# ctu-mrs/mrs_optic_flow

Measured on AMD Instinct MI355X. Metric: frame_pairs_per_s_fft_phase_corr, higher is better.
Workload: dtype f32

## Files before the change

### __graft_entry__.py

```python
from __future__ import annotations

import os
import subprocess
import sys

ROOT = os.path.dirname(os.path.abspath(__file__))


def build() -> None:
    jobs = f"-j{max(1, min(8, os.cpu_count() or 1))}"
    subprocess.check_call(["make", "-C", os.path.join(ROOT, "mrs_optic_flow_amd", "csrc"), "-s", jobs])
    subprocess.check_call(["make", "-C", os.path.join(ROOT, "oracle"), "-s", "all"])
    subprocess.check_call(["make", "-C", os.path.join(ROOT, "tests", "cpp"), "-s"])
    subprocess.check_call(["make", "-C", os.path.join(ROOT, "tests", "cpp_quality"), "-s"])
    subprocess.check_call(["make", "-C", os.path.join(ROOT, "tests", "cpp_gate"), "-s"])
    subprocess.check_call(["make", "-C", os.path.join(ROOT, "tests", "cpp_bm_quality"), "-s"])
    if ROOT not in sys.path:
        sys.path.insert(0, ROOT)
    import mrs_optic_flow_amd

    assert mrs_optic_flow_amd.FftMethod is not None
    subprocess.check_call([sys.executable, "-c", "from mrs_optic_flow_amd import _capi; _capi.load()"], cwd=ROOT,
                          env=dict(os.environ, MOF_NO_TORCH_PRELOAD="1"))


def smoke() -> None:
    if ROOT not in sys.path:
        sys.path.insert(0, ROOT)
    sys.path.insert(0, os.path.join(ROOT, "tests"))
    import torch
    import numpy as np

    import oracle_lib
    from mrs_optic_flow_amd import FastSpacedBMMethod, FftMethod, synth

    assert torch.cuda.is_available(), "smoke() needs a GPU"
    h, w = 160, 224
    cur, prev, shifts, _ = synth.batch_np(2, h, w, s=5, classes=False, k0=1)
    fm = FftMethod(sample_point_size=64, frame_shape=(h, w), grid=(3, 2), origin=(1, 1), stride=(79, 47))
    got = fm.process_batch_device(torch.from_numpy(cur).cuda(), torch.from_numpy(prev).cuda()).cpu().numpy()
    lay = oracle_lib.fft_layout(w, h, 64, 3, 2, (1, 1), (79, 47))
    for k in range(2):
        want, _ = oracle_lib.fft_process(cur[k], prev[k], lay, 64)
        assert np.allclose(got[k], want, rtol=0, atol=1e-4, equal_nan=True), (got[k], want)
        assert np.allclose(np.nanmedian(got[k], axis=0), shifts[k], rtol=0, atol=0.5)
    for n, gx, gy, stride in ((60, 3, 2, (70, 50)), (37, 4, 3, (40, 39))):
# ... 64 lines not shown
```

### mrs_optic_flow_amd/csrc/mof_capi.hip

```cpp

#include "mof.h"

#include <hip/hip_runtime.h>

#include <atomic>
#include <cmath>
#include <cstdarg>
#include <cstdio>
#include <cstdlib>
#include <cstring>
#include <memory>
#include <mutex>
#include <new>
#include <vector>

#include "capi_graph.hpp"
#include "host_pipe.hpp"
#include "mof_kernels.h"
#include "pc_launch.hpp"

#include "pc_gate_kernel.hip"

namespace {
thread_local char g_err[512] = "";
// ... 421 lines not shown
  if (c->peak_model == MOF_PEAK_OCL && c->search_radius < 0) return fail(MOF_ERR_BAD_ARG, "search_radius must be >= 0");
  return MOF_OK;
}

static void fft_destroy_now(void* p) {
  mof_fft_engine* e = static_cast<mof_fft_engine*>(p);
  mof::RelaxedCapture relaxed;
  (void)hipSetDevice(e->cfg.device);
  if (e->stream) (void)hipStreamSynchronize(e->stream);
  e->fence.wait_idle();
  e->gate_fence.wait_idle();
  delete e;
}
struct FftDestroyNow {
  void operator()(mof_fft_engine* e) const { fft_destroy_now(e); }
};

int mof_fft_create(const mof_fft_config* cfg, mof_fft_engine** out) try {
  if (!out) return fail(MOF_ERR_BAD_ARG, "null out");
  *out = nullptr;
  int rc = validate_fft(cfg);
  if (rc) return rc;
  rc = mof::select_device(cfg->device);
  if (rc) return rc;
  mof::RelaxedCapture relaxed;
  const size_t res = (size_t)cfg->grid_x * cfg->grid_y * 2;
  std::unique_ptr<mof_fft_engine, FftDestroyNow> e(new (std::nothrow) mof_fft_engine());
  if (!e) return fail(MOF_ERR_NO_MEMORY, "out of host memory");
  e->cfg = *cfg;
  e->frame_bytes = (size_t)cfg->frame_width * cfg->frame_height;
  if (!fft_route(*cfg, &e->plan, &e->route))
    return fail(MOF_ERR_UNSUPPORTED, "no plan for patch_size %d", cfg->patch_size);
  const FftRoute& r = e->route;
  const std::vector<float> tw = mof::twiddle_table(r.m);
  HIP_TRY(e->stream.create());
  HIP_TRY(mof::upload(e->d_twiddles, tw, e->stream));
  for (auto& frame : e->d_frames) {
    HIP_TRY(frame.alloc(e->frame_bytes));
    HIP_TRY(mof::fill_on(e->stream, frame, 0, e->frame_bytes));
  }
  HIP_TRY(mof::alloc_all(e->d_out, res, e->h_out, res, e->d_quality, res, e->h_quality, res, e->h_stage, e->frame_bytes));
  if (r.half_m > 0 || r.video == FftRoute::HALF_SEQ) HIP_TRY(mof::pc_configure_half(r.half_m > 0 ? r.half_m : r.video_m));
  if (r.family == FftRoute::LARGE) {
    HIP_TRY(e->fence.create());
    HIP_TRY(large_alloc(e.get(), cfg->grid_x * cfg->grid_y));
  } else if (r.family == FftRoute::PLANNED) {
    HIP_TRY(mof::pc_configure_generic());
  } else {
    HIP_TRY(mof::pc_configure(r.m));
  }
  if (r.video == FftRoute::SEQ) HIP_TRY(mof::pc_configure_sequence());
  if (r.video == FftRoute::SEQ_HALF) HIP_TRY(mof::pc_configure_sequence_half(r.m));
  *out = e.release();
  return MOF_OK;
} catch (const std::bad_alloc&) {
  return fail(MOF_ERR_NO_MEMORY, "mof_fft_create: out of host memory");
}

const char* mof_fft_kernel_variant(const mof_fft_engine* e) {
  if (!e) return "";
  const FftRoute& r = e->route;
  return r.half_m > 0 ? "planned-half"
                      : (r.family == FftRoute::LARGE ? "planned-large"
                                                     : (r.family == FftRoute::PLANNED ? "planned" : "stockham"));
}

void mof_fft_destroy(mof_fft_engine* e) {
// ... 650 lines not shown
```

### mrs_optic_flow_amd/csrc/mof_kernels.h

```cpp
#pragma once

#include <hip/hip_runtime.h>
#include <stdint.h>

#include <vector>

namespace mof {

struct PcArgs {
  const uint8_t* cur;
  const uint8_t* prev;
  size_t cur_stride;
  size_t prev_stride;
  size_t pitch;
  int grid_x, grid_y;
  int origin_x, origin_y;
  int stride_x, stride_y;
  int total;
  int stagger_div, stagger_units;
  int channels;
  int downscale;
  int peak_model;
  int search_radius;
  double max_px_speed_sq;
// ... 36 lines not shown
  int n_cand;
  const float* twiddles;
  int m, n;
  int mode;
  double M_log;
  double max_px_speed_sq;
  double* out;
  const int* flags;
  const float* cdc;
  int peak_model;
  int search_radius;
  double* quality;
  double min_response;
};
size_t pcl_zh_floats(const PcPlan& pl);
int pcl_candidates(const PcPlan& pl);
hipError_t launch_pcl_rows(const PclSrc& src, const PcPlan& pl, const float* twiddles, float* zh, size_t zh_stride, int* flags,
                           int n_images, int channels, int downscale, hipStream_t stream);
hipError_t launch_pcl_cols(const float* zh_prev, const float* zh_cur, size_t zh_stride, const PcPlan& pl, const float* twiddles,
                           float* Dt, float* cdc, const int* flags, int n_pairs, hipStream_t stream, int peak_model = 0);
hipError_t launch_pcl_peak(const PclFinal& a, const PcPlan& pl, int n_pairs, hipStream_t stream, bool candidates_done = false);
hipError_t launch_pcl_cdc(const float* zh_prev, const float* zh_cur, size_t zh_stride, int m, float* cdc, int n_pairs, hipStream_t stream);

bool pc_half_supported(int m);
int pc_half_workgroups_per_cu(int m);
hipError_t pc_configure_half(int m);
hipError_t launch_pc_half(const PcArgs& a, int m, int n, int n_pairs, hipStream_t stream);
bool pc_half_sequence_supported(int m);
hipError_t launch_pc_half_sequence(const PcArgs& a, int m, int n, int n_pairs, int run, hipStream_t stream);

bool pc_patch_size_supported(int n);
hipError_t pc_configure(int patch_size);
hipError_t launch_pc_field(const PcArgs& a, int patch_size, int n_pairs, hipStream_t stream);
bool pc_sequence_supported(int patch_size);
hipError_t pc_configure_sequence();
hipError_t launch_pc_sequence(const PcArgs& a, int n_pairs, int run, hipStream_t stream);
bool pc_sequence_half_supported(int patch_size);
hipError_t pc_configure_sequence_half(int patch_size);
hipError_t launch_pc_sequence_half(const PcArgs& a, int patch_size, int n_pairs, int run, hipStream_t stream);
hipError_t pc_configure_120();
hipError_t launch_pc_field_120(const PcArgs& a, int n_pairs, hipStream_t stream);
hipError_t launch_pc_response_gate(double* out, const double* quality, size_t n_patches, double min_response, hipStream_t stream);

struct BmArgs {
  const uint8_t* cur;
  const uint8_t* prev;
  size_t cur_stride, prev_stride, pitch;
  int grid_x, grid_y;
  int block, step, radius;
  int low_contrast_rule;
  int channels;
  int8_t* dx;
  int8_t* dy;
  int8_t* mode;
};

struct BmQArgs {
  uint32_t* quality = nullptr;
  uint32_t max_min_sad = 0xffffffffu, min_sad_range = 0u;
};
constexpr int BM_INVALID = -128;
inline bool bm_gate_armed(const BmQArgs& q) { return q.max_min_sad != 0xffffffffu || q.min_sad_range != 0u; }

bool bm_config_supported(int block, int radius);
bool bm_scan_plan(int block, int step, int radius, int grid_x, bool quality, int out[4]);
hipError_t launch_bm_scan(const BmArgs& a, const BmQArgs& q, int n_pairs, hipStream_t stream);
// ... 124 lines not shown
```

### mrs_optic_flow_amd/csrc/pc_common.hpp

```cpp
#pragma once

#include <hip/hip_runtime.h>
#include <stdint.h>

#include "mof_kernels.h"

namespace mof {
namespace {

struct cf {
  float x, y;
};

__device__ __forceinline__ cf cmul(cf a, cf b) { return {a.x * b.x - a.y * b.y, a.x * b.y + a.y * b.x}; }
__device__ __forceinline__ cf cadd(cf a, cf b) { return {a.x + b.x, a.y + b.y}; }
__device__ __forceinline__ cf csub(cf a, cf b) { return {a.x - b.x, a.y - b.y}; }
__device__ __forceinline__ cf mul_mi(cf a) { return {a.y, -a.x}; }

template <int R>
__device__ __forceinline__ void butterfly(cf* v);

template <>
__device__ __forceinline__ void butterfly<2>(cf* v) {
  cf a = v[0], b = v[1];
  v[0] = cadd(a, b);
  v[1] = csub(a, b);
}

template <>
__device__ __forceinline__ void butterfly<4>(cf* v) {
  cf a = cadd(v[0], v[2]), b = csub(v[0], v[2]);
  cf c = cadd(v[1], v[3]), d = mul_mi(csub(v[1], v[3]));
  v[0] = cadd(a, c);
  v[1] = cadd(b, d);
  v[2] = csub(a, c);
  v[3] = csub(b, d);
}

// ... 130 lines not shown
  const cf w[22] = {{1.f, 0.f}, {c1, -s1}, {c2, -s2}, {c3, -s3}, {h, -h}, {s3, -c3}, {s2, -c2}, {s1, -c1}, {0.f, -1.f},
                    {-s1, -c1}, {-s2, -c2}, {-s3, -c3}, {-h, -h}, {-c3, -s3}, {-c2, -s2}, {-c1, -s1}, {-1.f, 0.f},
                    {-c1, s1}, {-c2, s2}, {-c3, s3}, {-h, h}, {-s3, c3}};
  cf t[8][4];
#pragma unroll
  for (int n2 = 0; n2 < 8; ++n2) {
    cf a[4] = {v[n2], v[8 + n2], v[16 + n2], v[24 + n2]};
    butterfly<4>(a);
#pragma unroll
    for (int k1 = 0; k1 < 4; ++k1) t[n2][k1] = (n2 * k1 == 0) ? a[k1] : cmul(a[k1], w[n2 * k1]);
  }
#pragma unroll
  for (int k1 = 0; k1 < 4; ++k1) {
    cf b[8] = {t[0][k1], t[1][k1], t[2][k1], t[3][k1], t[4][k1], t[5][k1], t[6][k1], t[7][k1]};
    butterfly<8>(b);
#pragma unroll
    for (int k2 = 0; k2 < 8; ++k2) v[k1 + 4 * k2] = b[k2];
  }
}

__device__ __forceinline__ void wave_sync() {
  __builtin_amdgcn_fence(__ATOMIC_RELEASE, "wavefront");
  __builtin_amdgcn_wave_barrier();
  __builtin_amdgcn_fence(__ATOMIC_ACQUIRE, "wavefront");
}

__device__ __forceinline__ cf lds_read(const cf* p) {
  typedef float f2 __attribute__((ext_vector_type(2)));
  typedef const volatile f2 __attribute__((address_space(3))) * lds_f2_ptr;
  const f2 t = *(lds_f2_ptr)(p);
  return {t.x, t.y};
}

struct Best {
  float v;
  int idx;
};
__device__ __forceinline__ Best better(Best a, Best b) {
  return (b.v > a.v || (b.v == a.v && b.idx < a.idx)) ? b : a;
}

__device__ __forceinline__ int wave_lane() { return (int)__builtin_amdgcn_mbcnt_hi(~0u, __builtin_amdgcn_mbcnt_lo(~0u, 0u)); }

template <int OFF>
__device__ __forceinline__ uint32_t lane_xor(uint32_t x) {
  static_assert(OFF == 32 || OFF == 16 || OFF == 8 || OFF == 4 || OFF == 2 || OFF == 1, "one butterfly level");
  if constexpr (OFF == 32) {
    const auto r = __builtin_amdgcn_permlane32_swap(x, x, false, false);
    return (wave_lane() & 32) ? r[0] : r[1];
  } else if constexpr (OFF == 16) {
    const auto r = __builtin_amdgcn_permlane16_swap(x, x, false, false);
    return (wave_lane() & 16) ? r[0] : r[1];
  } else if constexpr (OFF == 8) {
    return (uint32_t)__builtin_amdgcn_update_dpp((int)x, (int)x, 0x128, 0xf, 0xf, false);
  } else if constexpr (OFF == 4) {
    const int lo = __builtin_amdgcn_update_dpp((int)x, (int)x, 0x104, 0xf, 0x5, false);
    return (uint32_t)__builtin_amdgcn_update_dpp(lo, (int)x, 0x114, 0xf, 0xa, false);
  } else if constexpr (OFF == 2) {
    return (uint32_t)__builtin_amdgcn_update_dpp((int)x, (int)x, 0x4e, 0xf, 0xf, false);
  } else {
    return (uint32_t)__builtin_amdgcn_update_dpp((int)x, (int)x, 0xb1, 0xf, 0xf, false);
  }
}
template <int OFF>
__device__ __forceinline__ int lane_xor(int x) { return (int)lane_xor<OFF>((uint32_t)x); }
template <int OFF>
__device__ __forceinline__ float lane_xor(float x) { return __uint_as_float(lane_xor<OFF>(__float_as_uint(x))); }
template <int OFF>
__device__ __forceinline__ double lane_xor(double x) {
  const uint64_t u = (uint64_t)__double_as_longlong(x);
  const uint32_t lo = lane_xor<OFF>((uint32_t)u), hi = lane_xor<OFF>((uint32_t)(u >> 32));
  return __longlong_as_double((long long)((uint64_t)hi << 32 | lo));
}
// ... 8 lines not shown
  v += lane_xor<1>(v);
  return v;
}
template <int OFF>
__device__ __forceinline__ void wave_sum3_level(double& a, double& b, double& c) {
  const double oa = lane_xor<OFF>(a), ob = lane_xor<OFF>(b), oc = lane_xor<OFF>(c);
  a += oa;
  b += ob;
  c += oc;
}
template <int TOP = 32>
__device__ __forceinline__ void wave_sum3(double& a, double& b, double& c) {
  if constexpr (TOP >= 32) wave_sum3_level<32>(a, b, c);
  if constexpr (TOP >= 16) wave_sum3_level<16>(a, b, c);
  wave_sum3_level<8>(a, b, c);
  wave_sum3_level<4>(a, b, c);
  wave_sum3_level<2>(a, b, c);
  wave_sum3_level<1>(a, b, c);
}
template <int OFF>
__device__ __forceinline__ Best wave_best_level(Best b) {
  const Best o = {lane_xor<OFF>(b.v), lane_xor<OFF>(b.idx)};
  return better(b, o);
}
__device__ __forceinline__ Best wave_best(Best b) {
  b = wave_best_level<32>(b);
  b = wave_best_level<16>(b);
  b = wave_best_level<8>(b);
  b = wave_best_level<4>(b);
  b = wave_best_level<2>(b);
  return wave_best_level<1>(b);
}

__device__ __forceinline__ uint32_t rgb2gray_fixed(uint32_t c0, uint32_t c1, uint32_t c2) {
  return (c0 * 4899u + c1 * 9617u + c2 * 1868u + 8192u) >> 14;
}

__device__ __forceinline__ uint32_t byte_at(const uint32_t* w, int i) { return (w[i >> 2] >> (8 * (i & 3))) & 0xffu; }
__device__ __forceinline__ uint32_t gray_at(const uint32_t* w, int i) { return rgb2gray_fixed(byte_at(w, i), byte_at(w, i + 1), byte_at(w, i + 2)); }
__device__ __forceinline__ uint32_t gray4_at(const uint32_t* w, int q) {
  uint32_t packed = 0;
#pragma unroll
  for (int b = 0; b < 4; ++b) packed |= gray_at(w, 3 * (4 * q + b)) << (8 * b);
  return packed;
}

__device__ __forceinline__ uint32_t gray4_from_bgr12(const uint8_t* p) {
  uint32_t w[3];
  __builtin_memcpy(w, p, 12);
  return gray4_at(w, 0);
}
__device__ __forceinline__ void gray16_from_bgr48(const uint8_t* p, uint32_t* g ) {
  uint32_t w[12];
  __builtin_memcpy(w, p, 48);
#pragma unroll
  for (int q = 0; q < 4; ++q) g[q] = gray4_at(w, q);
}
__device__ __forceinline__ void gray8_from_bgr24(const uint8_t* p, uint32_t* g ) {
  uint32_t w[6];
  __builtin_memcpy(w, p, 24);
#pragma unroll
  for (int q = 0; q < 2; ++q) g[q] = gray4_at(w, q);
}

template <int DS, int CH>
__device__ __forceinline__ uint32_t fetch_px(const uint8_t* __restrict__ base, size_t pitch, int y, int x) {
// ... 314 lines not shown
```

### mrs_optic_flow_amd/csrc/pc_kernel.hip

```cpp

#include <hip/hip_runtime.h>

#include <cmath>
#include <cstring>
#include <stdint.h>
#include <stdlib.h>

#include "mof_kernels.h"
#include "pc_common.hpp"
#include "pc_launch.hpp"

#include "pc_passes.hpp"
#include "pc_passes3.hpp"

namespace mof {

template <int N, int DS, int CH, int PK>
__global__ void __launch_bounds__(PcTraits<N>::T) pc_field_kernel(PcArgs a) {
  static_assert(CH == 1 || (CH == 3 && DS == 1), "BGR front end only for the full-resolution path");
  using P = PcTraits<N>;
  constexpr int T = P::T, H = N / 2, R1 = P::R1, R2 = P::R2, LPW = P::LPW;
  extern __shared__ __attribute__((aligned(16))) unsigned char smem[];
  cf* z = reinterpret_cast<cf*>(smem);
  Best* red = reinterpret_cast<Best*>(z + P::TILE);
  int* const_code = reinterpret_cast<int*>(red + 32);

  const int tid0 = threadIdx.x, lane0 = tid0 & 63, wave0 = tid0 >> 6;
  const int patches = a.grid_x * a.grid_y;
  constexpr int CPR = N / 16;
  const int lrow = wave0 * LPW + ord1<N>(lane0 / CPR), lcol = (lane0 % CPR) * 16;
  const bool ld_on = lane0 < LPW * CPR;

  constexpr bool PERSIST = P::PERSIST;
  constexpr bool FWD3 = N == 64 && DS == 1;
  constexpr bool RAW = (N == 128 || N == 64) && DS == 1;
  (void)patches;
  auto patch_base = [&](int p, const uint8_t* frames, size_t frame_stride) -> const uint8_t* {
    int pr, bx, by;
    if constexpr (PERSIST) {
      const int pt = p % patches;
      pr = p / patches;
      bx = pt % a.grid_x;
      by = pt / a.grid_x;
    } else {
      pr = blockIdx.z;
      bx = blockIdx.x;
      by = blockIdx.y;
    }
    const int px0 = a.origin_x + bx * a.stride_x, py0 = a.origin_y + by * a.stride_y;
    return frames + (size_t)pr * frame_stride + (size_t)(DS * py0) * a.pitch + (size_t)(CH * DS * px0);
  };

  cf tw_row[R2 - 1], tw_col[R2 - 1];
  {
    const int xr = lane0 % R1, xc = lane0 / (64 / R1);
#pragma unroll
    for (int k = 1; k < R2; ++k) {
      tw_row[k - 1] = {a.twiddles[2 * (k * xr)], a.twiddles[2 * (k * xr) + 1]};
      tw_col[k - 1] = {a.twiddles[2 * (k * xc)], a.twiddles[2 * (k * xc) + 1]};
    }
  }

  Fwd3Tw tw3;
  if constexpr (FWD3) tw3.load(a.twiddles, wave0, lane0);
  uint32_t cw[4] = {0u, 0u, 0u, 0u}, pw[4] = {0u, 0u, 0u, 0u};
  int p = PERSIST ? (int)blockIdx.x : (int)((blockIdx.z * gridDim.y + blockIdx.y) * gridDim.x + blockIdx.x);
  auto fetch16 = [&](int pp, uint32_t* c, uint32_t* q) {
    const uint8_t* cs = patch_base(pp, a.cur, a.cur_stride) + (size_t)lrow * a.pitch + CH * lcol;
    const uint8_t* ps = patch_base(pp, a.prev, a.prev_stride) + (size_t)lrow * a.pitch + CH * lcol;
    if constexpr (CH == 1) {
      __builtin_memcpy(c, cs, 16);
      __builtin_memcpy(q, ps, 16);
    } else {
      gray16_from_bgr48(cs, c);
      gray16_from_bgr48(ps, q);
    }
  };
  if (DS == 1 && p < a.total && ld_on) fetch16(p, cw, pw);
  if constexpr (PERSIST) {
    const int slot = (blockIdx.x / a.stagger_div) & 3;
    for (int i = 0; i < slot * a.stagger_units; ++i) __builtin_amdgcn_s_sleep(100);
  }
  for (; p < a.total; p += PERSIST ? (int)gridDim.x : a.total) {
  int lane = lane0, wave = wave0;
  asm volatile("" : "+v"(lane), "+v"(wave));
  lane &= 63;
  wave &= P::WAVES - 1;
  const int tid = wave * 64 + lane;
// ... 101 lines not shown
      constexpr int RPI = T / UPW;
      const int u = tid % UPW, vr = tid / UPW;
      const int um = (N - u) % N;
#pragma unroll
      for (int i = 0; i < (H - 1 + RPI - 1) / RPI; ++i) {
#pragma unroll
        for (int uu = 0; uu < N / UPW; ++uu) {
          const int v = 1 + vr + i * RPI;
          if (v < H) {
            const int uc = u + uu * UPW, umc = (N - uc) % N;
            (void)um;
            const cf zk = z[zaddr<N>(v, uc)], zm = z[zaddr<N>(N - v, umc)];
            const cf C = cross_power<PK>(zk, zm, false);
            z[zaddr<N>(v, uc)] = {C.x, -C.y};
          }
        }
      }
    }
    for (int u = tid; u <= H; u += T) {
      const int um = (N - u) % N;
      const bool self = (u == um);
      const cf C0 = cross_power<PK>(z[zaddr<N>(0, u)], z[zaddr<N>(0, um)], self);
      const cf Ch = cross_power<PK>(z[zaddr<N>(H, u)], z[zaddr<N>(H, um)], self);
      if (u == 0) *reinterpret_cast<float*>(const_code + 16) = C0.x;
      z[zaddr<N>(0, u)] = {C0.x + Ch.y, Ch.x - C0.y};
      if (!self) z[zaddr<N>(0, um)] = {C0.x - Ch.y, Ch.x + C0.y};
    }
  }
  __syncthreads();

  if (wave < P::WI) row_pass<N, P::LI>(z, wave * P::LI, lane, tw_row);
  }
  __syncthreads();
  Best best = {-__builtin_huge_valf(), 0x7fffffff};
  if (wave < P::WI) best = col_pass_inv<N, PK>(z, wave * P::LI, lane, tw_col, a.search_radius);
  best = wave_best(best);
  if (lane == 0) red[wave] = best;
  __syncthreads();

  float wval = 0.f;
  bool degenerate = false;
  if (wave == 0) {
    const int my_code = const_code[lane & 15];
    for (int w = 1; w < P::WAVES; ++w) best = better(best, red[w]);
    wval = centroid_window_value<N, PK>(best, lane, [&](int ys, int xs) {
      const int y = (ys + H) % N, x = (xs + H) % N;
      const cf s = z[zaddr<N>(y, x % H)];
      return x < H ? s.x : s.y;
    });
    degenerate = const_codes_degenerate<P::WAVES>(my_code, lane);
  }
  __syncthreads();
  if (wave == 0)
    centroid_gate_store<N, PK>(best, wval, lane, a.max_px_speed_sq, a.out + 2 * (size_t)p, a.quality ? a.quality + 2 * (size_t)p : nullptr, degenerate,
                               degenerate ? *reinterpret_cast<const float*>(const_code + 16) : 0.f);
  }
}

template <int N>
static hipError_t configure_n() {
  const size_t lds = PcTraits<N>::LDS_BYTES + pc_extra_lds();
  return pc_each_form([&](auto ds, auto ch, auto pk) { return pc_raise_lds(&pc_field_kernel<N, ds, ch, pk>, lds); });
}

template <int N>
static hipError_t launch_n(const PcArgs& a_in, int n_pairs, hipStream_t stream) {
  using Tr = PcTraits<N>;
  PcArgs a = a_in;
  a.total = n_pairs * a.grid_x * a.grid_y;
  const int cus = pc_cu_count();
  a.stagger_div = cus;
  {
    static const int units = [] { const char* e = getenv("MOF_PC_STAGGER"); return e ? atoi(e) : 0; }();
    a.stagger_units = units;
  }
  const dim3 b(Tr::T);
  const size_t lds = Tr::LDS_BYTES + pc_extra_lds();
  auto launch = [&](const PcArgs& aa, dim3 g) {
    return pc_dispatch_form(aa, [&](auto ds, auto ch, auto pk) {
      hipLaunchKernelGGL((pc_field_kernel<N, ds, ch, pk>), g, b, lds, stream, aa);
      return hipGetLastError();
    });
  };
  if constexpr (Tr::PERSIST) {
    const int per_cu = (int)((160u * 1024u) / lds);
    const int resident = cus * (per_cu < 1 ? 1 : (per_cu > 16 ? 16 : per_cu));
    return launch(a, dim3((unsigned)(a.total < resident ? a.total : resident)));
  } else {
    return pc_split_pairs(a, n_pairs, [&](const PcArgs& c, int nk) { return launch(c, dim3((unsigned)a.grid_x, (unsigned)a.grid_y, (unsigned)nk)); });
  }
}

hipError_t pc_configure(int patch_size) {
  switch (patch_size) {
    case 32: return configure_n<32>();
    case 64: return configure_n<64>();
    case 128: return configure_n<128>();
    case 120: return pc_configure_120();
    default: return hipErrorInvalidValue;
  }
}

hipError_t launch_pc_field(const PcArgs& a, int patch_size, int n_pairs, hipStream_t stream) {
  switch (patch_size) {
    case 32: return launch_n<32>(a, n_pairs, stream);
    case 64: return launch_n<64>(a, n_pairs, stream);
    case 128: return launch_n<128>(a, n_pairs, stream);
    case 120: return launch_pc_field_120(a, n_pairs, stream);
    default: return hipErrorInvalidValue;
  }
}

bool pc_patch_size_supported(int n) { return n == 32 || n == 64 || n == 128 || n == 120; }

}
```

### mrs_optic_flow_amd/csrc/pc_passes.hpp

```cpp
#pragma once

#include <hip/hip_runtime.h>
#include <stdint.h>

#include "mof_kernels.h"
#include "pc_common.hpp"

namespace mof {

namespace {

template <int N>
struct Cfg;
template <>
struct Cfg<32> {
  static constexpr int R1 = 8, R2 = 4, SK = 3, PITCH = 36;
};
template <>
struct Cfg<64> {
  static constexpr int R1 = 8, R2 = 8, SK = 3, PITCH = 72;
};
template <>
struct Cfg<128> {
  static constexpr int R1 = 16, R2 = 8, SK = 4, PITCH = 140;
};

template <int N>
__device__ __forceinline__ int ord1(int j) {
  if constexpr (N == 128) return 2 * (j & 3) + (j >> 2);
  else return j;
}
template <int N>
__device__ __forceinline__ int ord2(int j) {
  if constexpr (N == 128) return ((j & 1) << 2) | (j & 2) | (j >> 2);
  else return j;
}

}

template <int N>
struct PcTraits {
  static constexpr int T = N * N / 16;
  static constexpr int WAVES = T / 64;
  static constexpr int LPW = N / WAVES;
  static constexpr int R1 = Cfg<N>::R1, R2 = Cfg<N>::R2, SK = Cfg<N>::SK, PITCH = Cfg<N>::PITCH;
  static constexpr int BMIN = R1 < R2 ? R1 : R2;
  static constexpr int LI = (LPW / 2 > 64 / BMIN) ? LPW / 2 : 64 / BMIN;
  static constexpr int WI = (N / 2) / LI;
  static constexpr int TILE = N * PITCH + (N == 128 ? 24 : 0) + (N == 64 ? 56 : 0);
  static constexpr size_t LDS_BYTES = sizeof(float) * 2 * (size_t)TILE + 64 * sizeof(Best);
  static constexpr bool PERSIST = N >= 128;
  static constexpr bool FUSE_XPOW = N <= 64;
  static_assert(R1 * R2 == N && T % 64 == 0 && 64 % R1 == 0 && 64 % R2 == 0, "bad plan");
};

template <int N>
__device__ __forceinline__ int zaddr(int r, int c) {
  if constexpr (N == 128) return r * PcTraits<N>::PITCH + 8 * (r >> 5) + c + (c >> PcTraits<N>::SK);
  else if constexpr (N == 64) return r * PcTraits<N>::PITCH + 8 * (r >> 3) + c + (c >> PcTraits<N>::SK);
  else return r * PcTraits<N>::PITCH + c + (c >> PcTraits<N>::SK);
}

template <int N>
struct RawCfg {
  static constexpr int PITCH = 2 * N + 16, CPR = N / 16;
};
template <int N>
__device__ __forceinline__ unsigned char* raw_area(cf* z, int line0) {
  return reinterpret_cast<unsigned char*>(z + zaddr<N>(line0, 0));
}
__device__ __forceinline__ uint32_t lds_read_u16(const unsigned char* p) {
  typedef const volatile uint16_t __attribute__((address_space(3))) * lds_u16_ptr;
  return *(lds_u16_ptr)(p);
}
template <int N>
__device__ __forceinline__ void raw_store(cf* z, int line0, int lane, const uint32_t* cw, const uint32_t* pw) {
  typedef uint32_t u4 __attribute__((ext_vector_type(4)));
  typedef u4 __attribute__((address_space(3))) * lds_u4_ptr;
  unsigned char* dst = raw_area<N>(z, line0) + (lane / RawCfg<N>::CPR) * RawCfg<N>::PITCH + (lane % RawCfg<N>::CPR) * 32;
  u4 lo, hi;
  lo.x = __builtin_amdgcn_perm(pw[0], cw[0], 0x05010400u);
  lo.y = __builtin_amdgcn_perm(pw[0], cw[0], 0x07030602u);
  lo.z = __builtin_amdgcn_perm(pw[1], cw[1], 0x05010400u);
  lo.w = __builtin_amdgcn_perm(pw[1], cw[1], 0x07030602u);
  hi.x = __builtin_amdgcn_perm(pw[2], cw[2], 0x05010400u);
  hi.y = __builtin_amdgcn_perm(pw[2], cw[2], 0x07030602u);
  hi.z = __builtin_amdgcn_perm(pw[3], cw[3], 0x05010400u);
// ... 187 lines not shown
#pragma unroll
    for (int b = 0; b < PER; ++b) {
      const int col = col0 + lane % CW + CW * b, x = ord1<N>(lane / CW);
#pragma unroll
      for (int k = 0; k < R1; ++k) z[zaddr<N>(x * R1 + k, col)] = v[b][k];
    }
    wave_sync();
  }
  {
    constexpr int PER = LPW * R1 / 64, CW = 64 / R1;
    cf v[PER][R2];
#pragma unroll
    for (int b = 0; b < PER; ++b) {
      const int col = col0 + lane % CW + CW * b, x = lane / CW;
#pragma unroll
      for (int k = 0; k < R2; ++k) {
        cf a = lds_read(&z[zaddr<N>(x + k * R1, col)]);
        v[b][k] = (k == 0 || R2 == 8) ? a : cmul(a, tw_col[k - 1]);
      }
      if constexpr (R2 == 8) butterfly8_tw(v[b], tw_col);
      else butterfly<R2>(v[b]);
    }
    wave_sync();
#pragma unroll
    for (int b = 0; b < PER; ++b) {
      const int col = col0 + lane % CW + CW * b, x = lane / CW;
#pragma unroll
      for (int k = 0; k < R2; ++k) z[zaddr<N>(x + k * R1, col)] = v[b][k];
    }
    wave_sync();
  }
}

template <int N, int PK>
__device__ __forceinline__ Best col_pass_inv(cf* __restrict__ z, int col0, int lane, const cf* tw_col, int search_radius) {
  using P = PcTraits<N>;
  constexpr int R1 = P::R1, R2 = P::R2, LI = P::LI, H = N / 2;
  {
    constexpr int PER = LI * R2 / 64, CW = 64 / R2;
    static_assert(PER >= 1, "inverse column stage 1 does not fill the wave");
    cf v[PER][R1];
#pragma unroll
    for (int b = 0; b < PER; ++b) {
      const int col = col0 + lane % CW + CW * b, x = ord1<N>(lane / CW);
      static_assert(R1 % 2 == 0 && 64 / CW == R2, "row classes below assume x < R2 and an even R1");
      const bool x0 = x == 0;
#pragma unroll
      for (int k = 0; k < R1; ++k) {
        const int r = x + k * R2;
        const int rr = (k < R1 / 2) ? r : ((k == R1 / 2 && x0) ? 0 : N - r);
        const cf a = lds_read(&z[zaddr<N>(rr, col)]), c = lds_read(&z[zaddr<N>(rr, col + H)]);
        cf e;
        if (k < R1 / 2) {
          e = {a.x - c.y, a.y + c.x};
          if (k == 0 && x0) e = {a.x, c.x};
        } else {
          e = {a.x + c.y, c.x - a.y};
          if (k == R1 / 2 && x0) e = {a.y, c.y};
        }
        v[b][k] = e;
      }
      butterfly<R1>(v[b]);
    }
    wave_sync();
#pragma unroll
    for (int b = 0; b < PER; ++b) {
      const int col = col0 + lane % CW + CW * b, x = ord1<N>(lane / CW);
#pragma unroll
      for (int k = 0; k < R1; ++k) z[zaddr<N>(x * R1 + k, col)] = v[b][k];
    }
    wave_sync();
  }
  Best best = {-__builtin_huge_valf(), 0x7fffffff};
  {
    constexpr int PER = LI * R1 / 64, CW = 64 / R1;
    cf v[PER][R2];
#pragma unroll
    for (int b = 0; b < PER; ++b) {
      const int col = col0 + lane % CW + CW * b, x = lane / CW;
#pragma unroll
      for (int k = 0; k < R2; ++k) {
        cf a = lds_read(&z[zaddr<N>(x + k * R1, col)]);
        v[b][k] = (k == 0 || R2 == 8) ? a : cmul(a, tw_col[k - 1]);
      }
      if constexpr (R2 == 8) butterfly8_tw(v[b], tw_col);
      else butterfly<R2>(v[b]);
      if constexpr (PK == 1) {
#pragma unroll
        for (int k = 0; k < R2; ++k) {
          const int y = x + k * R1;
          v[b][k].x = ocl_scale_mask<N>(v[b][k].x, y, col, search_radius);
          v[b][k].y = ocl_scale_mask<N>(v[b][k].y, y, col + H, search_radius);
        }
      }
    }
    wave_sync();
    float m = -__builtin_huge_valf();
#pragma unroll
    for (int b = 0; b < PER; ++b)
#pragma unroll
      for (int k = 0; k < R2; ++k) m = fmaxf(m, fmaxf(v[b][k].x, v[b][k].y));
    int mi = 0x7fffffff;
#pragma unroll
    for (int b = 0; b < PER; ++b) {
      const int col = col0 + lane % CW + CW * b, x = lane / CW;
#pragma unroll
      for (int k = 0; k < R2; ++k) {
        const int y = x + k * R1;
        z[zaddr<N>(y, col)] = v[b][k];
        const int base = ((y + H) % N) * N + col;
        mi = min(mi, v[b][k].x == m ? base + H : 0x7fffffff);
        mi = min(mi, v[b][k].y == m ? base : 0x7fffffff);
      }
    }
    best = Best{m, mi};
  }
  return best;
}

}
```

### mrs_optic_flow_amd/csrc/pc_passes3.hpp

```cpp
#pragma once

#include "pc_passes.hpp"

namespace mof {

struct Fwd3Tw {
  cf wr[3], wc[3];
  __device__ __forceinline__ void load(const float* __restrict__ table, int wave, int lane) {
    const int k1 = 4 * wave + (lane & 3), m2 = lane >> 2;
#pragma unroll
    for (int i = 1; i < 4; ++i) {
      wr[i - 1] = {table[2 * (i * k1)], table[2 * (i * k1) + 1]};
      wc[i - 1] = {table[2 * (i * m2)], table[2 * (i * m2) + 1]};
    }
  }
};

__device__ __forceinline__ int t3addr(int y, int b, int k1) { return 68 * y + 4 * (y >> 4) + 17 * b + k1; }

__device__ __forceinline__ void fwd3_rows(cf* __restrict__ z, int wave, int lane) {
  constexpr int N = 64;
  const int slot = lane >> 2, n2 = lane & 3, y = 16 * wave + slot;
  const unsigned char* src = raw_area<N>(z, 16 * wave) + slot * RawCfg<N>::PITCH + 2 * n2;
  cf v[16];
#pragma unroll
  for (int n1 = 0; n1 < 16; ++n1) {
    const uint32_t cp = lds_read_u16(src + 8 * n1);
    v[n1] = {(float)(cp & 0xffu), (float)(cp >> 8)};
  }
  butterfly<16>(v);
  wave_sync();
#pragma unroll
  for (int k1 = 0; k1 < 16; ++k1) z[t3addr(y, n2, k1)] = v[k1];
}

__device__ __forceinline__ void fwd3_mid(cf* __restrict__ z, int wave, int lane, const Fwd3Tw& tw) {
  const int k1 = 4 * wave + (lane & 3), m2 = lane >> 2;
  cf e[4][4];
#pragma unroll
  for (int m1 = 0; m1 < 4; ++m1)
#pragma unroll
    for (int n2 = 0; n2 < 4; ++n2) e[m1][n2] = lds_read(&z[t3addr(m2 + 16 * m1, n2, k1)]);
#pragma unroll
  for (int m1 = 0; m1 < 4; ++m1) {
    cf t[4] = {e[m1][0], cmul(e[m1][1], tw.wr[0]), cmul(e[m1][2], tw.wr[1]), cmul(e[m1][3], tw.wr[2])};
    butterfly<4>(t);
#pragma unroll
// ... 31 lines not shown
```

### mrs_optic_flow_amd/csrc/wave_selftest.hip

```cpp
#include <hip/hip_runtime.h>
#include <stdint.h>

#include "dev_mem.hpp"
#include "pc_common.hpp"

namespace mof {
namespace {

__device__ __forceinline__ bool same_bits(double a, double b) { return __double_as_longlong(a) == __double_as_longlong(b); }
__device__ __forceinline__ bool same_bits(float a, float b) { return __float_as_uint(a) == __float_as_uint(b); }

template <int OFF>
__device__ __forceinline__ int check_xor(int lane) {
  const uint32_t u = 0x9e3779b9u * (uint32_t)(lane + 1) ^ (uint32_t)lane << 24;
  const int i = (int)~u;
  const float f = (float)(lane - 31) * 1.25f;
  const double d = __longlong_as_double((long long)((uint64_t)(0x3ff00000u + (uint32_t)lane * 0x1357u) << 32 | u));
  int bad = 0;
  bad += lane_xor<OFF>(u) != (uint32_t)__shfl_xor((int)u, OFF, 64);
  bad += lane_xor<OFF>(i) != __shfl_xor(i, OFF, 64);
  bad += !same_bits(lane_xor<OFF>(f), __shfl_xor(f, OFF, 64));
  bad += !same_bits(lane_xor<OFF>(d), __shfl_xor(d, OFF, 64));
  return bad;
}

__device__ __forceinline__ int check_best(float v, int lane, Best* lds) {
  const Best raw = {v, lane * 3 + 5};
  const Best mine = better(Best{-__builtin_huge_valf(), 0x7fffffff}, raw);
  lds[lane] = mine;
  wave_sync();
  Best ref = lds[0];
#pragma unroll 1
  for (int l = 1; l < 64; ++l) ref = better(ref, lds[l]);
  wave_sync();
  const Best got = wave_best(mine);
  int bad = (!same_bits(got.v, ref.v)) + (got.idx != ref.idx);
  Best old = raw;
#pragma unroll
  for (int off = 32; off > 0; off >>= 1) {
    const Best o = {__shfl_xor(old.v, off, 64), __shfl_xor(old.idx, off, 64)};
    old = better(old, o);
  }
  const Best neu = wave_best(raw);
  return bad + (!same_bits(neu.v, old.v)) + (neu.idx != old.idx);
}

template <int TOP>
__device__ __forceinline__ int check_sum3(int n, int lane) {
  const double val = lane < n ? (double)((lane % 7 - 3) * 1.0e-3f + 1.0f / (float)(lane + 1)) * ((lane & 5) == 1 ? -4096.0 : 1.0) : 0.0;
  double cx = (double)(lane % 7 - 3) * val, cy = (double)(lane / 7 + 29) * val, sum = val;
  double rx = cx, ry = cy, rs = sum;
  wave_sum3<TOP>(cx, cy, sum);
#pragma unroll
  for (int off = TOP; off > 0; off >>= 1) {
    rx += __shfl_xor(rx, off, 64);
    ry += __shfl_xor(ry, off, 64);
    rs += __shfl_xor(rs, off, 64);
  }
  int bad = (!same_bits(cx, rx)) + (!same_bits(cy, ry)) + (!same_bits(sum, rs));
  bad += !same_bits(wave_sum<TOP>(val), rs);
  return bad;
}

__global__ __launch_bounds__(64) void wave_ops_selftest_kernel(int* mismatches) {
  __shared__ Best lds[64];
  const int lane = (int)threadIdx.x;
  const float ninf = -__builtin_huge_valf(), nan = __builtin_nanf("");
  int bad = 0;
  bad += check_xor<32>(lane) + check_xor<16>(lane) + check_xor<8>(lane) + check_xor<4>(lane) + check_xor<2>(lane) + check_xor<1>(lane);
  bad += check_best((float)((lane * 37) % 64) - 20.5f, lane, lds);
  bad += check_best(lane == 9 || lane == 13 ? 7.f : (float)(lane % 5), lane, lds);
  bad += check_best(lane == 40 || lane == 3 ? 7.f : (float)(lane % 5), lane, lds);
  bad += check_best(ninf, lane, lds);
  bad += check_best(lane == 21 ? nan : (float)(63 - lane), lane, lds);
  {
    bad += check_best(nan, lane, lds);
    bad += wave_best(better(Best{ninf, 0x7fffffff}, Best{nan, lane})).idx != 0x7fffffff;
  }
  bad += check_sum3<32>(25, lane) + check_sum3<32>(49, lane) + check_sum3<16>(25, lane);
  if (bad) atomicAdd(mismatches, bad);
}

}
}

extern "C" int mof_selftest_wave_ops(void) {
  mof::DevMem<int> d;
  int h = -1;
  if (d.alloc(1) != hipSuccess) return -1;
  bool ok = hipMemset(d, 0, sizeof(int)) == hipSuccess;
  if (ok) {
    hipLaunchKernelGGL(mof::wave_ops_selftest_kernel, dim3(1), dim3(64), 0, 0, d.get());
    ok = hipGetLastError() == hipSuccess && hipMemcpy(&h, d, sizeof(int), hipMemcpyDeviceToHost) == hipSuccess;
  }
  return ok ? h : -1;
}
```

Baseline: 1.774 million.

## Split inverse argmax into value-first max and rare index pass; pack twiddle rows

The inverse column pass now first computes only the per-lane peak value. A wave max and a cross-wave max over LDS follow, and the first-index search runs only in waves that actually hold the global peak, keeping the transformed values in registers for that pass. Twiddle factors for each row are precomputed on the host and appended to the table so kernels load them with 16-byte vector loads instead of gathered scalar loads. Mirrored-row LDS addressing in the inverse stage is simplified, and one barrier is dropped on the value-first path. The cost is extra registers to hold values and a new path whose correctness rests on exact float equality for index recovery.

```diff
diff --git a/__graft_entry__.py b/__graft_entry__.py
--- a/__graft_entry__.py
+++ b/__graft_entry__.py
@@ -12,6 +12,7 @@
     subprocess.check_call(["make", "-C", os.path.join(ROOT, "mrs_optic_flow_amd", "csrc"), "-s", jobs])
     subprocess.check_call(["make", "-C", os.path.join(ROOT, "oracle"), "-s", "all"])
     subprocess.check_call(["make", "-C", os.path.join(ROOT, "tests", "cpp"), "-s"])
+    subprocess.check_call(["make", "-C", os.path.join(ROOT, "tests", "cpp"), "-s", "-f", "argmax_select.mk"])
     subprocess.check_call(["make", "-C", os.path.join(ROOT, "tests", "cpp_quality"), "-s"])
     subprocess.check_call(["make", "-C", os.path.join(ROOT, "tests", "cpp_gate"), "-s"])
     subprocess.check_call(["make", "-C", os.path.join(ROOT, "tests", "cpp_bm_quality"), "-s"])
diff --git a/mrs_optic_flow_amd/csrc/mof_capi.hip b/mrs_optic_flow_amd/csrc/mof_capi.hip
--- a/mrs_optic_flow_amd/csrc/mof_capi.hip
+++ b/mrs_optic_flow_amd/csrc/mof_capi.hip
@@ -477,7 +477,8 @@
   if (!fft_route(*cfg, &e->plan, &e->route))
     return fail(MOF_ERR_UNSUPPORTED, "no plan for patch_size %d", cfg->patch_size);
   const FftRoute& r = e->route;
-  const std::vector<float> tw = mof::twiddle_table(r.m);
+  std::vector<float> tw = mof::twiddle_table(r.m);
+  mof::pc_append_twiddle_rows(tw, r.m);
   HIP_TRY(e->stream.create());
   HIP_TRY(mof::upload(e->d_twiddles, tw, e->stream));
   for (auto& frame : e->d_frames) {
diff --git a/mrs_optic_flow_amd/csrc/mof_kernels.h b/mrs_optic_flow_amd/csrc/mof_kernels.h
--- a/mrs_optic_flow_amd/csrc/mof_kernels.h
+++ b/mrs_optic_flow_amd/csrc/mof_kernels.h
@@ -92,6 +92,7 @@
 bool pc_patch_size_supported(int n);
 hipError_t pc_configure(int patch_size);
 hipError_t launch_pc_field(const PcArgs& a, int patch_size, int n_pairs, hipStream_t stream);
+void pc_append_twiddle_rows(std::vector<float>& table, int n);
 bool pc_sequence_supported(int patch_size);
 hipError_t pc_configure_sequence();
 hipError_t launch_pc_sequence(const PcArgs& a, int n_pairs, int run, hipStream_t stream);
diff --git a/mrs_optic_flow_amd/csrc/pc_argmax.hpp b/mrs_optic_flow_amd/csrc/pc_argmax.hpp
--- /dev/null
+++ b/mrs_optic_flow_amd/csrc/pc_argmax.hpp
@@ -0,0 +1,30 @@
+#pragma once
+
+#if defined(__HIPCC__)
+#define MOF_ARGMAX_FN __host__ __device__ __forceinline__
+#else
+#define MOF_ARGMAX_FN inline
+#endif
+
+namespace mof {
+namespace {
+
+struct Best {
+  float v;
+  int idx;
+};
+MOF_ARGMAX_FN Best better(Best a, Best b) {
+  return (b.v > a.v || (b.v == a.v && b.idx < a.idx)) ? b : a;
+}
+
+MOF_ARGMAX_FN Best argmax_neutral() { return Best{-__builtin_huge_valf(), 0x7fffffff}; }
+
+MOF_ARGMAX_FN int argmax_first_index(int mi, float cand, float m, int idx) {
+  const int c = cand == m ? idx : 0x7fffffff;
+  return mi < c ? mi : c;
+}
+
+MOF_ARGMAX_FN Best argmax_entry(float m, float gm, int mi) { return m == gm ? Best{m, mi} : argmax_neutral(); }
+
+}
+}
diff --git a/mrs_optic_flow_amd/csrc/pc_common.hpp b/mrs_optic_flow_amd/csrc/pc_common.hpp
--- a/mrs_optic_flow_amd/csrc/pc_common.hpp
+++ b/mrs_optic_flow_amd/csrc/pc_common.hpp
@@ -4,6 +4,7 @@
 #include <stdint.h>
 
 #include "mof_kernels.h"
+#include "pc_argmax.hpp"
 
 namespace mof {
 namespace {
@@ -200,13 +201,6 @@
   return {t.x, t.y};
 }
 
-struct Best {
-  float v;
-  int idx;
-};
-__device__ __forceinline__ Best better(Best a, Best b) {
-  return (b.v > a.v || (b.v == a.v && b.idx < a.idx)) ? b : a;
-}
 
 __device__ __forceinline__ int wave_lane() { return (int)__builtin_amdgcn_mbcnt_hi(~0u, __builtin_amdgcn_mbcnt_lo(~0u, 0u)); }
 
@@ -281,6 +275,21 @@
   return wave_best_level<1>(b);
 }
 
+__device__ __forceinline__ float wave_max(float v) {
+  {
+    const auto r = __builtin_amdgcn_permlane32_swap(__float_as_uint(v), __float_as_uint(v), false, false);
+    v = fmaxf(__uint_as_float(r[0]), __uint_as_float(r[1]));
+  }
+  {
+    const auto r = __builtin_amdgcn_permlane16_swap(__float_as_uint(v), __float_as_uint(v), false, false);
+    v = fmaxf(__uint_as_float(r[0]), __uint_as_float(r[1]));
+  }
+  v = fmaxf(v, lane_xor<8>(v));
+  v = fmaxf(v, lane_xor<4>(v));
+  v = fmaxf(v, lane_xor<2>(v));
+  return fmaxf(v, lane_xor<1>(v));
+}
+
 __device__ __forceinline__ uint32_t rgb2gray_fixed(uint32_t c0, uint32_t c1, uint32_t c2) {
   return (c0 * 4899u + c1 * 9617u + c2 * 1868u + 8192u) >> 14;
 }
diff --git a/mrs_optic_flow_amd/csrc/pc_kernel.hip b/mrs_optic_flow_amd/csrc/pc_kernel.hip
--- a/mrs_optic_flow_amd/csrc/pc_kernel.hip
+++ b/mrs_optic_flow_amd/csrc/pc_kernel.hip
@@ -34,6 +34,7 @@
   constexpr bool PERSIST = P::PERSIST;
   constexpr bool FWD3 = N == 64 && DS == 1;
   constexpr bool RAW = (N == 128 || N == 64) && DS == 1;
+  constexpr bool VALUE_FIRST = !PERSIST && P::WAVES > 1;
   (void)patches;
   auto patch_base = [&](int p, const uint8_t* frames, size_t frame_stride) -> const uint8_t* {
     int pr, bx, by;
@@ -54,6 +55,10 @@
   cf tw_row[R2 - 1], tw_col[R2 - 1];
   {
     const int xr = lane0 % R1, xc = lane0 / (64 / R1);
+    if constexpr (TwRows<N>::USE) {
+      tw_row_load<R2>(a.twiddles + TwRows<N>::ROWS_AT + 2 * R2 * xr, tw_row);
+      tw_row_load<R2>(a.twiddles + TwRows<N>::ROWS_AT + 2 * R2 * xc, tw_col);
+    } else
 #pragma unroll
     for (int k = 1; k < R2; ++k) {
       tw_row[k - 1] = {a.twiddles[2 * (k * xr)], a.twiddles[2 * (k * xr) + 1]};
@@ -221,10 +226,28 @@
   if (wave < P::WI) row_pass<N, P::LI>(z, wave * P::LI, lane, tw_row);
   }
   __syncthreads();
-  Best best = {-__builtin_huge_valf(), 0x7fffffff};
+  Best best = argmax_neutral();
+  if constexpr (VALUE_FIRST) {
+    static_assert(P::WI == P::WAVES, "every wave runs the inverse column pass");
+    float* red_max = reinterpret_cast<float*>(red + 16);
+    cf sv[InvPlan<N>::PER * R2];
+    const float m = col_pass_inv<N, PK, false>(z, wave * P::LI, lane, tw_col, a.search_radius, sv).v;
+    const float wm = wave_max(m);
+    if (lane == 0) red_max[wave] = wm;
+    __syncthreads();
+    float gm = red_max[0];
+#pragma unroll
+    for (int w = 1; w < P::WAVES; ++w) gm = fmaxf(gm, red_max[w]);
+    if (__builtin_amdgcn_ballot_w64(m == gm) != 0ull) {
+      asm volatile("");
+      best = wave_best(argmax_entry(m, gm, col_pass_inv_index<N>(sv, m, wave * P::LI, lane)));
+    }
+    if (lane == 0) red[wave] = best;
+  } else {
   if (wave < P::WI) best = col_pass_inv<N, PK>(z, wave * P::LI, lane, tw_col, a.search_radius);
   best = wave_best(best);
   if (lane == 0) red[wave] = best;
+  }
   __syncthreads();
 
   float wval = 0.f;
@@ -239,7 +262,7 @@
     });
     degenerate = const_codes_degenerate<P::WAVES>(my_code, lane);
   }
-  __syncthreads();
+  if constexpr (!VALUE_FIRST) __syncthreads();
   if (wave == 0)
     centroid_gate_store<N, PK>(best, wval, lane, a.max_px_speed_sq, a.out + 2 * (size_t)p, a.quality ? a.quality + 2 * (size_t)p : nullptr, degenerate,
                                degenerate ? *reinterpret_cast<const float*>(const_code + 16) : 0.f);
@@ -302,4 +325,25 @@
 
 bool pc_patch_size_supported(int n) { return n == 32 || n == 64 || n == 128 || n == 120; }
 
-}
+template <int N>
+static void append_rows_n(std::vector<float>& t) {
+  using R = TwRows<N>;
+  t.resize(R::FLOATS);
+  auto copy = [&](size_t at, int k) {
+    t[at] = t[2 * (size_t)k];
+    t[at + 1] = t[2 * (size_t)k + 1];
+  };
+  for (int x = 0; x < R::R1; ++x)
+    for (int k = 0; k < R::R2; ++k) copy(R::ROWS_AT + 2 * (size_t)(x * R::R2 + k), k * x);
+  if constexpr (N == 64)
+    for (int i = 0; i < 16; ++i)
+      for (int k = 0; k < 4; ++k) copy(R::FWD3_AT + 2 * (size_t)(i * 4 + k), k * i);
+}
+
+void pc_append_twiddle_rows(std::vector<float>& table, int n) {
+  if (table.size() != 2 * (size_t)n) return;
+  if (n == 32) append_rows_n<32>(table);
+  else if (n == 64) append_rows_n<64>(table);
+}
+
+}
diff --git a/mrs_optic_flow_amd/csrc/pc_passes.hpp b/mrs_optic_flow_amd/csrc/pc_passes.hpp
--- a/mrs_optic_flow_amd/csrc/pc_passes.hpp
+++ b/mrs_optic_flow_amd/csrc/pc_passes.hpp
@@ -53,6 +53,25 @@
   static constexpr bool FUSE_XPOW = N <= 64;
   static_assert(R1 * R2 == N && T % 64 == 0 && 64 % R1 == 0 && 64 % R2 == 0, "bad plan");
 };
+
+template <int N>
+struct TwRows {
+  static constexpr int R1 = Cfg<N>::R1, R2 = Cfg<N>::R2;
+  static constexpr int ROWS_AT = 2 * N;
+  static constexpr int FWD3_AT = ROWS_AT + 2 * R1 * R2;
+  static constexpr int FLOATS = FWD3_AT + (N == 64 ? 2 * 16 * 4 : 0);
+  static constexpr bool USE = N <= 64;
+  static_assert((R1 - 1) * (R2 - 1) < N && R2 % 2 == 0, "rows are copies of the classic table, whole 16-byte pieces");
+};
+template <int R>
+__device__ __forceinline__ void tw_row_load(const float* __restrict__ row, cf* tw) {
+  typedef float f4 __attribute__((ext_vector_type(4)));
+  f4 q[R / 2];
+#pragma unroll
+  for (int j = 0; j < R / 2; ++j) q[j] = reinterpret_cast<const f4*>(row)[j];
+#pragma unroll
+  for (int k = 1; k < R; ++k) tw[k - 1] = (k & 1) ? cf{q[k / 2].z, q[k / 2].w} : cf{q[k / 2].x, q[k / 2].y};
+}
 
 template <int N>
 __device__ __forceinline__ int zaddr(int r, int c) {
@@ -306,8 +325,40 @@
   }
 }
 
-template <int N, int PK>
-__device__ __forceinline__ Best col_pass_inv(cf* __restrict__ z, int col0, int lane, const cf* tw_col, int search_radius) {
+template <int N>
+struct InvMirror {
+  static constexpr int R1 = Cfg<N>::R1, R2 = Cfg<N>::R2, PITCH = Cfg<N>::PITCH, STEP = 8;
+  static constexpr bool USE = N <= 64;
+  static constexpr int rskew(int r) { return N == 128 ? 8 * (r >> 5) : (N == 64 ? 8 * (r >> 3) : 0); }
+  static constexpr int off(int k) { return (N - k * R2) * PITCH + rskew(N - k * R2 - 1); }
+  static constexpr int cls(int k) { return rskew(N - k * R2) != rskew(N - k * R2 - 1) ? 1 : 0; }
+  static constexpr bool holds() {
+    for (int x = 0; x < R2; ++x)
+      for (int k = R1 / 2; k < R1; ++k) {
+        if (k == R1 / 2 && x == 0) continue;
+        const int r = N - x - k * R2;
+        if (r * PITCH + rskew(r) != off(k) - x * PITCH + (x == 0 && cls(k) == 1 ? STEP : 0)) return false;
+        if (rskew(N - k * R2) - rskew(N - k * R2 - 1) != (cls(k) ? STEP : 0)) return false;
+      }
+    return true;
+  }
+};
+
+template <int N>
+struct InvPlan {
+  static constexpr int PER = PcTraits<N>::LI * PcTraits<N>::R1 / 64;
+};
+
+template <int N>
+__device__ __forceinline__ int inv_index_step(int mi, cf v, float m, int y, int col) {
+  constexpr int H = N / 2;
+  const int base = ((y + H) % N) * N + col;
+  mi = argmax_first_index(mi, v.x, m, base + H);
+  return argmax_first_index(mi, v.y, m, base);
+}
+
+template <int N, int PK, bool INDEX = true>
+__device__ __forceinline__ Best col_pass_inv(cf* __restrict__ z, int col0, int lane, const cf* tw_col, int search_radius, cf* keep = nullptr) {
   using P = PcTraits<N>;
   constexpr int R1 = P::R1, R2 = P::R2, LI = P::LI, H = N / 2;
   {
@@ -319,6 +370,28 @@
       const int col = col0 + lane % CW + CW * b, x = ord1<N>(lane / CW);
       static_assert(R1 % 2 == 0 && 64 / CW == R2, "row classes below assume x < R2 and an even R1");
       const bool x0 = x == 0;
+      if constexpr (InvMirror<N>::USE) {
+        static_assert(R2 <= 8 && 8 % R2 == 0 && H % (1 << P::SK) == 0 && InvMirror<N>::holds(), "stage-1 address offsets of the mirror rows");
+        constexpr int HOFF = H + (H >> P::SK);
+        const int ccol = col + (col >> P::SK), mrow = ccol - x * P::PITCH;
+        const int mbase[2] = {mrow, mrow + (x0 ? InvMirror<N>::STEP : 0)};
+#pragma unroll
+        for (int k = 0; k < R1; ++k) {
+          int at = zaddr<N>(x + k * R2, col);
+          if (k >= R1 / 2) at = mbase[InvMirror<N>::cls(k)] + InvMirror<N>::off(k);
+          if (k == R1 / 2) at = x0 ? ccol : at;
+          const cf a = lds_read(&z[at]), c = lds_read(&z[at + HOFF]);
+          cf e;
+          if (k < R1 / 2) {
+            e = {a.x - c.y, a.y + c.x};
+            if (k == 0 && x0) e = {a.x, c.x};
+          } else {
+            e = {a.x + c.y, c.x - a.y};
+            if (k == R1 / 2 && x0) e = {a.y, c.y};
+          }
+          v[b][k] = e;
+        }
+      } else {
 #pragma unroll
       for (int k = 0; k < R1; ++k) {
         const int r = x + k * R2;
@@ -334,6 +407,7 @@
         }
         v[b][k] = e;
       }
+      }
       butterfly<R1>(v[b]);
     }
     wave_sync();
@@ -347,7 +421,7 @@
   }
   Best best = {-__builtin_huge_valf(), 0x7fffffff};
   {
-    constexpr int PER = LI * R1 / 64, CW = 64 / R1;
+    constexpr int PER = InvPlan<N>::PER, CW = 64 / R1;
     cf v[PER][R2];
 #pragma unroll
     for (int b = 0; b < PER; ++b) {
@@ -382,9 +456,12 @@
       for (int k = 0; k < R2; ++k) {
         const int y = x + k * R1;
         z[zaddr<N>(y, col)] = v[b][k];
-        const int base = ((y + H) % N) * N + col;
-        mi = min(mi, v[b][k].x == m ? base + H : 0x7fffffff);
-        mi = min(mi, v[b][k].y == m ? base : 0x7fffffff);
+        if constexpr (INDEX) {
+          const int base = ((y + H) % N) * N + col;
+          mi = min(mi, v[b][k].x == m ? base + H : 0x7fffffff);
+          mi = min(mi, v[b][k].y == m ? base : 0x7fffffff);
+        }
+        else keep[b * R2 + k] = v[b][k];
       }
     }
     best = Best{m, mi};
@@ -392,4 +469,16 @@
   return best;
 }
 
-}
+template <int N>
+__device__ __forceinline__ int col_pass_inv_index(const cf* keep, float m, int col0, int lane) {
+  using P = PcTraits<N>;
+  constexpr int R1 = P::R1, R2 = P::R2, PER = InvPlan<N>::PER, CW = 64 / R1;
+  int mi = 0x7fffffff;
+#pragma unroll
+  for (int b = 0; b < PER; ++b)
+#pragma unroll
+    for (int k = 0; k < R2; ++k) mi = inv_index_step<N>(mi, keep[b * R2 + k], m, lane / CW + k * R1, col0 + lane % CW + CW * b);
+  return mi;
+}
+
+}
diff --git a/mrs_optic_flow_amd/csrc/pc_passes3.hpp b/mrs_optic_flow_amd/csrc/pc_passes3.hpp
--- a/mrs_optic_flow_amd/csrc/pc_passes3.hpp
+++ b/mrs_optic_flow_amd/csrc/pc_passes3.hpp
@@ -8,11 +8,9 @@
   cf wr[3], wc[3];
   __device__ __forceinline__ void load(const float* __restrict__ table, int wave, int lane) {
     const int k1 = 4 * wave + (lane & 3), m2 = lane >> 2;
-#pragma unroll
-    for (int i = 1; i < 4; ++i) {
-      wr[i - 1] = {table[2 * (i * k1)], table[2 * (i * k1) + 1]};
-      wc[i - 1] = {table[2 * (i * m2)], table[2 * (i * m2) + 1]};
-    }
+    static_assert(TwRows<64>::USE, "the packed rows are behind the classic table");
+    tw_row_load<4>(table + TwRows<64>::FWD3_AT + 8 * k1, wr);
+    tw_row_load<4>(table + TwRows<64>::FWD3_AT + 8 * m2, wc);
   }
 };
 
diff --git a/mrs_optic_flow_amd/csrc/wave_selftest.hip b/mrs_optic_flow_amd/csrc/wave_selftest.hip
--- a/mrs_optic_flow_amd/csrc/wave_selftest.hip
+++ b/mrs_optic_flow_amd/csrc/wave_selftest.hip
@@ -45,6 +45,20 @@
   return bad + (!same_bits(neu.v, old.v)) + (neu.idx != old.idx);
 }
 
+__device__ __forceinline__ int check_max(float v, int lane, Best* lds) {
+  lds[lane] = Best{v, lane};
+  wave_sync();
+  float ref = lds[0].v;
+#pragma unroll 1
+  for (int l = 1; l < 64; ++l) ref = fmaxf(ref, lds[l].v);
+  wave_sync();
+  float old = v;
+#pragma unroll
+  for (int off = 32; off > 0; off >>= 1) old = fmaxf(old, __shfl_xor(old, off, 64));
+  const float got = wave_max(v);
+  return !(got == ref) + !(got == old);
+}
+
 template <int TOP>
 __device__ __forceinline__ int check_sum3(int n, int lane) {
   const double val = lane < n ? (double)((lane % 7 - 3) * 1.0e-3f + 1.0f / (float)(lane + 1)) * ((lane & 5) == 1 ? -4096.0 : 1.0) : 0.0;
@@ -77,6 +91,12 @@
     bad += check_best(nan, lane, lds);
     bad += wave_best(better(Best{ninf, 0x7fffffff}, Best{nan, lane})).idx != 0x7fffffff;
   }
+  bad += check_max((float)((lane * 37) % 64) - 20.5f, lane, lds);
+  bad += check_max((float)(((lane + 32) * 37) % 64) - 20.5f, lane, lds);
+  bad += check_max(lane == 40 || lane == 3 ? 7.f : (float)(lane % 5), lane, lds);
+  bad += check_max(lane == 17 ? 0.f : (lane == 50 ? -0.f : -1.f - (float)lane), lane, lds);
+  bad += check_max(ninf, lane, lds);
+  bad += check_max(lane == 63 ? -3.e38f : ninf, lane, lds);
   bad += check_sum3<32>(25, lane) + check_sum3<32>(49, lane) + check_sum3<16>(25, lane);
   if (bad) atomicAdd(mismatches, bad);
 }
```

New measurement: 1.839 million (median of 6 runs). 1.04x the previous value.
